# icameling/lidar_camera_calibration

Measured on AMD Instinct MI355X. Metric: chessboard-corner frames/sec + max corner error (mm), VLP-16 cloud, higher is better.
Workload: dtype f32

## Files before the change

lidar_camera_calibration_amd/csrc/ilcc_internal.h:

```cpp
#pragma once

#include <hip/hip_runtime.h>
#include <stdint.h>

#include "ilcc_hip.h"

#define ILCC_WAVE 64

namespace ilcc {

constexpr int kCropThreads = 256;
constexpr int kCropChunk = 4096;
#ifndef ILCC_K2_THREADS
#define ILCC_K2_THREADS 256
#endif
constexpr int kFrameThreads = ILCC_K2_THREADS;
#ifndef ILCC_K3_THREADS
#define ILCC_K3_THREADS 256
#endif
#ifndef ILCC_K45_THREADS
#define ILCC_K45_THREADS 256
#endif
constexpr int kPlaneThreads = ILCC_K3_THREADS;
constexpr int kPlaneThreadsSmallBatch = 1024;
#ifndef ILCC_SMALL_BATCH
#define ILCC_SMALL_BATCH 64
#endif
constexpr int kSmallBatchFrames = ILCC_SMALL_BATCH;
constexpr int kHistThreads = ILCC_K45_THREADS;
constexpr int kWalkThreads = 256;
#ifndef ILCC_K6_THREADS
#define ILCC_K6_THREADS 256
#endif
constexpr int kGridThreads = ILCC_K6_THREADS;
#ifndef ILCC_K6_THREADS_LARGE
#define ILCC_K6_THREADS_LARGE 512
#endif
constexpr int kGridThreadsLarge = ILCC_K6_THREADS_LARGE;
#ifndef ILCC_K6_LARGE_FROM
#define ILCC_K6_LARGE_FROM 2048
#endif
constexpr int kGridLargeFrom = ILCC_K6_LARGE_FROM;
constexpr int kTileA = 4;
#ifndef ILCC_TILE_B
#define ILCC_TILE_B 4
#endif
constexpr int kTileB = ILCC_TILE_B;
#ifndef ILCC_K6_GROUP
#define ILCC_K6_GROUP 7
#endif
constexpr int kThetaGroup = ILCC_K6_GROUP;
constexpr int kGridLdsPointsMax = 8192;
constexpr int kGridTableMax = 8192;
#ifndef ILCC_K7_THREADS
#define ILCC_K7_THREADS 256
#endif
constexpr int kSolveThreads = ILCC_K7_THREADS;
#ifndef ILCC_K7R_THREADS
#define ILCC_K7R_THREADS 192
#endif
constexpr int kRefineThreads = ILCC_K7R_THREADS;
constexpr int kRefineThreadsSmallBatch = 768;
constexpr int kRefineList = 32;
constexpr int kTieCap = 256;
constexpr float kTieEps = 2e-5f;
constexpr int kCoverageCellsMax = 1024;
constexpr int kIterSlots = 64;
constexpr int kBatchWords = 3 * kIterSlots + 2;
constexpr int kClusterHashSize = 1 << 17;
constexpr int kClusterLdsPointsMax = 4096;
constexpr int kClusterLdsPointsMin = 1024;
constexpr int kClusterCellsMin = 512;
constexpr int kClusterCellsMax = 6144;

struct GridPartial {
  float cost;
  uint32_t d2;
  uint32_t flat;
  uint32_t pad;
};

struct SolveRec {
  double x[3];
  double cost_a, cost_b, sel;
  double margin;
  int32_t iters_a, iters_b, phase, valid;
  int32_t flags, ties;
};

struct RefineOut {
  long long cost_q, alt_q;
  int32_t lat[3];
  int32_t phase, rounds, hops;
};

struct GridTables {
  const float* cth;
  const float* sth;
  const float* ay;
  const float* az;
  int32_t n_th, n_ty, n_tz;
  int32_t c_th, c_ty, c_tz;
};

struct SeedMap {
  int32_t stride_t, stride_th, off_th;
};

struct GridSeed {
  const GridPartial* records;
  uint32_t blocks;
  SeedMap map;
};

struct GridPass {
  GridTables t;
  GridPartial* out;
  uint32_t blocks;
  uint32_t walk_limit;
  uint32_t* bound;
  GridSeed seed;
  int32_t window_tiles, radius_th, step_th;
  uint32_t collect_ties;
  uint32_t box_points;
  uint32_t* grp_alive;
  uint32_t* grp_mask;
  uint32_t grp_count, grp_words;
};

struct Ctx {
  const float4* xyzi;
  const uint64_t* off;
  const float* clicks;
  uint32_t n_frames;
  uint32_t crop_chunks;
  ilcc_result* res;
  float4* roi;
  float4* cluster;
  float4* board;
  float4* pca;
  float4* optim;
  float2* yz;
  uint8_t* lab;
  uint32_t* n_lab;
  uint32_t* walk_stride;
  float2* walk_yz;
  uint8_t* walk_lab;
  uint32_t *walk_mi, *walk_nrim;
  uint8_t* cls;
  uint32_t* crop_counts;
  unsigned long long* crop_masks;
  uint32_t* uf_parent;
  uint32_t* uf_count;
  uint32_t* uf_hash_head;
  uint32_t* uf_hash_next;
  uint32_t cluster_lds_points;
  uint32_t cluster_cells_cap;
  uint32_t wide;
  uint32_t cluster_bits;
  uint32_t online_tier;
  float online_window;
  uint32_t* frame_flags;
  uint32_t* n_finite;
  uint32_t* crop_fin;
  uint32_t* list_count;
  uint32_t* list;
  void* list_frames;
  uint32_t list_grid;
  GridPartial* partial;
  SolveRec* solve_rec;
  uint32_t grid_blocks;
  uint32_t grid_lds_points;
  uint32_t* grid_bound;
  uint32_t* grid_bound_sub;
  uint32_t* tie_count;
  GridPartial* tie_list;
  unsigned long long* grid_iters;
  GridTables grid;
  const double2* th_lattice;
  int32_t th_lat_lo, th_lat_hi;
  int32_t refine_hop_y, refine_hop_z;
  ilcc_params p;
};

__host__ __device__ inline uint32_t walk_stride(uint32_t M) {
  if (M <= 2) return 1u;
  uint32_t S = ((uint32_t)((float)M * 0.6180339f)) | 1u;
  for (;; S += 2u) {
    uint32_t a = S, b = M;
    while (b) {
      const uint32_t t = a % b;
      a = b;
      b = t;
    }
    if (a == 1u) break;
  }
  return S >= M ? 1u : S;
}

__device__ __forceinline__ int lane_id() { return threadIdx.x & (ILCC_WAVE - 1); }
__device__ __forceinline__ int wave_id() { return threadIdx.x >> 6; }

template <typename T>
__device__ __forceinline__ T wave_sum(T v) {
#pragma unroll
  for (int o = ILCC_WAVE / 2; o > 0; o >>= 1) v += __shfl_down(v, o, ILCC_WAVE);
  return v;
}

template <typename T>
__device__ __forceinline__ T block_sum(T v, T* scratch) {
  v = wave_sum(v);
  const int nw = (blockDim.x + ILCC_WAVE - 1) / ILCC_WAVE;
  __syncthreads();
  if (lane_id() == 0) scratch[wave_id()] = v;
  __syncthreads();
// ... 90 lines not shown
```

lidar_camera_calibration_amd/csrc/k7_refine_corners.hip:

```cpp
#include "ilcc_internal.h"

namespace ilcc {

struct Divisor {
  double d, y;
};
__device__ __forceinline__ Divisor make_divisor(double d) { return Divisor{d, 1.0 / d}; }
__device__ __forceinline__ double div_by(double a, const Divisor& v) {
  const double q = a * v.y;
  const double r = __builtin_fma(-q, v.d, a);
  return __builtin_fma(r, v.y, q);
}

struct Board {
  double W, H, g, delta;
};
struct SolveBoard {
  double W, H, delta;
  double Wg2, Hg2;
  Divisor g;
};
__device__ __forceinline__ SolveBoard make_board(const ilcc_params& p) {
  SolveBoard b;
  b.W = (double)p.board_w;
// ... 531 lines not shown
      if (rel < 0.25) s.radius *= 0.5;
      if (rel > 0.75) s.radius = fmax(s.radius, 3.0 * s.step_norm);
      if (s.radius > 1e16) s.radius = 1e16;
      s.mu = fmax(1e-8, 2.0 * s.mu / 10.0);
      s.reuse = 0;
    } else {
      s.radius *= 0.5;
      s.reuse = 1;
    }
  }
  final_cost = x_cost;
  return iter;
}

__device__ __forceinline__ bool partial_less(const GridPartial& a, const GridPartial& b) {
  return a.cost < b.cost || (a.cost == b.cost && (a.d2 < b.d2 || (a.d2 == b.d2 && a.flat < b.flat)));
}

template <bool WIDE>
__device__ __forceinline__ void solve_wave(const Ctx& c, Problem& q, uint32_t f, uint32_t slot, SolveRec* out, Dog& dog) {
  double x[3] = {0.0, 0.0, 0.0};
  int phase = (int)slot;
  if (c.p.phase_mode != 2) {
    phase = (c.p.phase_mode == 1) ? 1 : 0;
  }
  q.tlw = phase != 0;
  double cost[2] = {0.0, 0.0};
  int iters[2] = {0, 0};
#pragma nounroll
  for (int pass = 0; pass < 2; ++pass) {
    q.oob = pass == 0;
    double fc = 0.0;
    const int it = trust_region_minimize<WIDE>(q, x, fc, c.p.max_iterations, dog);
    cost[pass] = fc;
    iters[pass] = it;
  }
#ifdef ILCC_K7_TIMING
  if (blockIdx.x == 0 && threadIdx.x == 0) {
    printf("K7a f0 slot %d: iters %d + %d; cycles dogleg %llu, evaluate<false> %llu, evaluate<true> %llu\n", (int)slot, iters[0], iters[1], g_k7_t[0], g_k7_t[1], g_k7_t[2]);
    g_k7_t[0] = g_k7_t[1] = g_k7_t[2] = 0;
  }
#endif
  q.oob = true;
  double cs[10];
  evaluate<false, WIDE>(q, x, cs);
  if (WIDE ? threadIdx.x == 0 : lane_id() == 0) {
    out->x[0] = x[0];
    out->x[1] = x[1];
    out->x[2] = x[2];
    out->cost_a = cost[0];
    out->cost_b = cost[1];
    out->sel = cs[0];
    out->iters_a = iters[0];
    out->iters_b = iters[1];
    out->phase = phase;
    out->valid = 1;
    out->margin = 0.0;
    out->flags = 0;
    out->ties = 0;
  }
}

#ifndef ILCC_K7A_WAVES_PER_EU
#define ILCC_K7A_WAVES_PER_EU 3
#endif
__global__ __launch_bounds__(kSolveThreads) __attribute__((amdgpu_waves_per_eu(ILCC_K7A_WAVES_PER_EU, ILCC_K7A_WAVES_PER_EU))) void k7a_local_solve(Ctx c, SolveRec* rec, int n_slots) {
  extern __shared__ __align__(16) unsigned char smem[];
  __shared__ Dog s_dog[kSolveWaves];
  const uint32_t wave = (uint32_t)wave_id();
  const uint32_t solve = blockIdx.x * (uint32_t)kSolveWaves + wave;
  const uint32_t f = solve / (uint32_t)n_slots, slot = solve % (uint32_t)n_slots;
  const bool live = f < c.n_frames && c.res[f].status == ILCC_OK;
  const uint32_t n = live ? c.n_lab[f] : 0u;
  const bool in_lds = n <= c.grid_lds_points;
  const uint32_t local_frame = wave / (uint32_t)n_slots;
  float2* s_yz = reinterpret_cast<float2*>(smem) + (size_t)local_frame * c.grid_lds_points;
  uint8_t* s_lab = smem + sizeof(float2) * (size_t)c.grid_lds_points * (size_t)(kSolveWaves / n_slots) + (size_t)local_frame * c.grid_lds_points;
  const uint64_t beg = live ? c.off[f] : 0u;
  if (live && in_lds) {
    for (uint32_t i = slot * ILCC_WAVE + (uint32_t)lane_id(); i < n; i += (uint32_t)n_slots * ILCC_WAVE) {
      s_yz[i] = c.yz[beg + i];
      s_lab[i] = c.lab[beg + i];
    }
  }
  __syncthreads();
  if (f >= c.n_frames) return;
  SolveRec* out = &rec[2 * f + slot];
  if (!live) {
    if (lane_id() == 0) out->valid = 0;
    return;
  }
  Problem q;
  q.n = n;
  q.bd = make_board(c.p);
  if (in_lds) {
    q.yz = s_yz;
    q.lab = s_lab;
    solve_wave<false>(c, q, f, slot, out, s_dog[wave]);
  } else {
    q.yz = c.yz + beg;
    q.lab = c.lab + beg;
    solve_wave<false>(c, q, f, slot, out, s_dog[wave]);
  }
}

__global__ __launch_bounds__(kSolveThreads) void k7a_local_solve_wide(Ctx c, SolveRec* rec) {
  extern __shared__ __align__(16) unsigned char smem[];
  __shared__ double s_red[2 * kSolveRedDoubles];
  __shared__ Dog s_dog[kSolveWaves];
  const uint32_t f = blockIdx.x, slot = blockIdx.y;
  SolveRec* out = &rec[2 * f + slot];
  if (c.res[f].status != ILCC_OK) {
    if (threadIdx.x == 0) out->valid = 0;
    return;
  }
  float2* s_yz = reinterpret_cast<float2*>(smem);
  uint8_t* s_lab = smem + sizeof(float2) * (size_t)c.grid_lds_points;
  const uint64_t beg = c.off[f];
  const uint32_t n = c.n_lab[f];
  int flip = 0;
  Problem q;
  q.n = n;
  q.bd = make_board(c.p);
  q.red = s_red;
  q.flip = &flip;
  if (n <= c.grid_lds_points) {
    for (uint32_t i = threadIdx.x; i < n; i += blockDim.x) {
      s_yz[i] = c.yz[beg + i];
      s_lab[i] = c.lab[beg + i];
    }
    __syncthreads();
    q.yz = s_yz;
    q.lab = s_lab;
    solve_wave<true>(c, q, f, slot, out, s_dog[wave_id()]);
  } else {
    q.yz = c.yz + beg;
    q.lab = c.lab + beg;
    solve_wave<true>(c, q, f, slot, out, s_dog[wave_id()]);
  }
}

constexpr double kCostQOne = 1099511627776.0;
#define kRefineWaves ((int)(blockDim.x >> 6))
static_assert(kRefineThreads % ILCC_WAVE == 0 && kRefineThreads / ILCC_WAVE >= 3 && kRefineThreads >= kRefineList &&
              kRefineThreadsSmallBatch % (3 * ILCC_WAVE) == 0,
              "ILCC_K7R_THREADS must be a multiple of 64, at least 192");
constexpr float kBorderRisk = 4e-6f;
constexpr int32_t kNoTheta = INT32_MIN;

struct RCand {
  int32_t q0, q1, q2, phase;
};
constexpr int kRefineWavesMax = kRefineThreadsSmallBatch / ILCC_WAVE;
constexpr int kActQueue = 128;
struct RefineShared {
  RCand cand[kRefineList];
  GridPartial meta[kRefineList];
  unsigned long long acc[3][kRefineList];
  uint32_t queue[kRefineWavesMax][kActQueue];
};

struct RefineState {
  int32_t lat[3];
  int32_t phase, rounds, hops, capped;
  int32_t skip_first;
  long long cost, alt;
};

struct AxisTerms {
  double in_dist;
  double out_dist;
  bool inside;
  bool odd;
};
__device__ __forceinline__ AxisTerms axis_terms(double v, double n) {
  AxisTerms t;
  t.inside = v > 0 && v < n;
  const double fl = floor(v);
  t.odd = (((int)fl) & 1) != 0;
  const double fr = v - fl;
  t.in_dist = (fr > 0.5) ? (fl + 1.0) - v : fr;
  t.out_dist = fmin(fabs(v), fabs(v - n));
  return t;
}
__device__ __forceinline__ double term_q(const AxisTerms& ai, const AxisTerms& aj, bool tlw, bool laser_white, double delta) {
#ifndef ILCC_K7R_BRANCHFREE
#define ILCC_K7R_BRANCHFREE 0
#endif
  double res = 0.0;
  if (ILCC_K7R_BRANCHFREE) {
    const bool white = tlw != (ai.odd != aj.odd);
    const double in_sum = ai.in_dist + aj.in_dist, out_sum = ai.out_dist + aj.out_dist;
    res = (ai.inside && aj.inside) ? ((laser_white != white) ? in_sum : 0.0) : out_sum;
  } else if (ai.inside && aj.inside) {
    const bool white = (ai.odd == aj.odd) ? tlw : !tlw;
    if (laser_white != white) res = ai.in_dist + aj.in_dist;
  } else {
    res = ai.out_dist + aj.out_dist;
  }
  const double r0 = (res > delta) ? 2.0 * delta * res - delta * delta : res * res;
  return rint(r0 * (0.5 * kCostQOne));
}

__device__ __forceinline__ int refine_sweep(const Ctx& c, const Board& bd, const float2* yz, const uint8_t* lab, uint32_t n,
                                            RefineShared& sh, int n_cand, int& sweep) {
  const int buf = sweep % 3;
  if (threadIdx.x < kRefineList) sh.acc[(sweep + 1) % 3][threadIdx.x] = 0ull;
  __syncthreads();
  const int lane = lane_id();
  const int slices = ILCC_WAVE / n_cand;
  const int cand = lane % n_cand, slice = lane / n_cand;
  if (slice < slices) {
    const RCand cd = sh.cand[cand];
    if (cd.q0 != kNoTheta) {
      const double div = (double)(c.p.refine_div > 0 ? c.p.refine_div : 1);
      const double2 cs = c.th_lattice[cd.q0 - c.th_lat_lo];
      const double x1 = c.p.ty_min + (double)cd.q1 * (c.p.ty_step / div), x2 = c.p.tz_min + (double)cd.q2 * (c.p.tz_step / div);
      const double inv_g = 1.0 / bd.g;
      const bool tlw = cd.phase != 0;
      long long sum = 0;
      for (uint32_t p = (uint32_t)(wave_id() * slices + slice); p < n; p += (uint32_t)(kRefineWaves * slices)) {
        const float2 v = yz[p];
        const double y = (double)v.x, z = (double)v.y;
        const double ry = cs.x * y - cs.y * z;
        const double rz = cs.y * y + cs.x * z;
        const AxisTerms ai = axis_terms(((ry + x1) + bd.W * bd.g / 2.0) * inv_g, bd.W);
        const AxisTerms aj = axis_terms(((rz + x2) + bd.H * bd.g / 2.0) * inv_g, bd.H);
        sum += (long long)term_q(ai, aj, tlw, lab[p] != 0, bd.delta);
      }
      atomicAdd(&sh.acc[buf][cand], (unsigned long long)sum);
    }
  }
  __syncthreads();
  ++sweep;
  return buf;
}

__device__ __forceinline__ int stencil_sweep(const Ctx& c, const Board& bd, const float2* yz, const uint8_t* lab, uint32_t n,
                                             RefineShared& sh, int n_th, const int32_t th[3], const int32_t ty[3],
                                             const int32_t tz[3], int phase, bool parity, int& sweep) {
  const int buf = sweep % 3;
  if (threadIdx.x < kRefineList) sh.acc[(sweep + 1) % 3][threadIdx.x] = 0ull;
  __syncthreads();
  const int wid = __builtin_amdgcn_readfirstlane(wave_id());
  const int waves_per_theta = kRefineWaves / n_th;
  const int it = wid % n_th, grp = wid / n_th;
  const int32_t q0 = th[it];
  if (grp < waves_per_theta && q0 != kNoTheta) {
    const int lane = lane_id();
    const double div = (double)(c.p.refine_div > 0 ? c.p.refine_div : 1);
    const double2 cs = c.th_lattice[q0 - c.th_lat_lo];
    double x1[3], x2[3];
#pragma unroll
    for (int k = 0; k < 3; ++k) {
      x1[k] = c.p.ty_min + (double)ty[k] * (c.p.ty_step / div);
      x2[k] = c.p.tz_min + (double)tz[k] * (c.p.tz_step / div);
    }
    const double inv_g = 1.0 / bd.g;
    double acc[9];
#pragma unroll
    for (int e = 0; e < 9; ++e) acc[e] = 0.0;
    auto eval_point = [&](uint32_t p) {
      const float2 v = yz[p];
      const bool laser_white = lab[p] != 0;
      const double y = (double)v.x, z = (double)v.y;
      const double ry = cs.x * y - cs.y * z;
      const double rz = cs.y * y + cs.x * z;
      AxisTerms ai[3], aj[3];
#pragma unroll
      for (int k = 0; k < 3; ++k) {
        ai[k] = axis_terms(((ry + x1[k]) + bd.W * bd.g / 2.0) * inv_g, bd.W);
        aj[k] = axis_terms(((rz + x2[k]) + bd.H * bd.g / 2.0) * inv_g, bd.H);
      }
#pragma unroll
      for (int a = 0; a < 3; ++a)
#pragma unroll
        for (int b = 0; b < 3; ++b) {
          const bool tlw = ((phase ^ (parity ? ((a + b) & 1) : 0)) != 0);
          acc[a * 3 + b] += term_q(ai[a], aj[b], tlw, laser_white, bd.delta);
        }
    };
    const uint32_t n_slices = (uint32_t)(waves_per_theta * ILCC_WAVE);
    const bool skip_silent = !parity && ty[0] <= ty[1] && ty[1] <= ty[2] && tz[0] <= tz[1] && tz[1] <= tz[2] && c.p.ty_step > 0.0 && c.p.tz_step > 0.0;
    if (skip_silent) {
      uint32_t* queue = sh.queue[wid];
      uint32_t head = 0, tail = 0;
      const bool tlw0 = phase != 0;
      for (uint32_t base = (uint32_t)(grp * ILCC_WAVE); base < n; base += n_slices) {
        const uint32_t p = base + (uint32_t)lane;
        bool active = false;
        if (p < n) {
          const float2 v = yz[p];
          const double y = (double)v.x, z = (double)v.y;
          const double ry = cs.x * y - cs.y * z;
          const double rz = cs.y * y + cs.x * z;
          const double i0 = ((ry + x1[0]) + bd.W * bd.g / 2.0) * inv_g, i2 = ((ry + x1[2]) + bd.W * bd.g / 2.0) * inv_g;
          const double j0 = ((rz + x2[0]) + bd.H * bd.g / 2.0) * inv_g, j2 = ((rz + x2[2]) + bd.H * bd.g / 2.0) * inv_g;
          const double fi = floor(i0), fj = floor(j0);
          const bool one_cell = i0 > 0 && i2 < bd.W && j0 > 0 && j2 < bd.H && fi == floor(i2) && fj == floor(j2);
          const bool odd_i = (((int)fi) & 1) != 0, odd_j = (((int)fj) & 1) != 0;
          const bool white = (odd_i == odd_j) ? tlw0 : !tlw0;
          active = !(one_cell && (lab[p] != 0) == white);
        }
        const unsigned long long m = __ballot(active);
        if (m != 0ull) {
          if (active) queue[(tail + (uint32_t)__popcll(m & ((1ull << lane) - 1ull))) & (kActQueue - 1)] = p;
          tail += (uint32_t)__popcll(m);
          __builtin_amdgcn_fence(__ATOMIC_RELEASE, "wavefront");
          __builtin_amdgcn_wave_barrier();
          __builtin_amdgcn_fence(__ATOMIC_ACQUIRE, "wavefront");
          while (tail - head >= (uint32_t)ILCC_WAVE) {
            eval_point(queue[(head + (uint32_t)lane) & (kActQueue - 1)]);
            head += ILCC_WAVE;
          }
          __builtin_amdgcn_fence(__ATOMIC_RELEASE, "wavefront");
          __builtin_amdgcn_wave_barrier();
        }
      }
      if ((uint32_t)lane < tail - head) eval_point(queue[(head + (uint32_t)lane) & (kActQueue - 1)]);
    } else {
      for (uint32_t p = (uint32_t)(grp * ILCC_WAVE + lane); p < n; p += n_slices) eval_point(p);
    }
#pragma unroll
    for (int e = 0; e < 9; ++e) {
      unsigned long long t = (unsigned long long)(long long)acc[e];
      t += xor_lane_u64<8>(t);
      t += xor_lane_u64<4>(t);
      t += xor_lane_u64<2>(t);
      t += xor_lane_u64<1>(t);
      if ((lane & 15) == 0) atomicAdd(&sh.acc[buf][it * 9 + e], t);
    }
  }
  __syncthreads();
  ++sweep;
  return buf;
}

__device__ void pattern_refine(const Ctx& c, const Board& bd, const float2* yz, const uint8_t* lab, uint32_t n,
                               RefineShared& sh, int& sweep, RefineState& st) {
  const bool refine = c.p.refine_div > 0;
  const int div = refine ? c.p.refine_div : 1;
  st.rounds = 0;
  st.hops = 0;
  st.capped = 0;
  st.cost = 0;
  st.alt = 0;
  for (;;) {
    int stride = div, r = 0;
    if (st.skip_first && refine && div >= 2 && c.p.refine_max_rounds >= 1) {
      stride = div >> 1;
      r = 1;
    }
    st.skip_first = 0;
    while (refine && stride >= 1 && r < c.p.refine_max_rounds) {
      int32_t th[3], ty[3], tz[3];
#pragma unroll
      for (int k = 0; k < 3; ++k) {
        const int q0 = st.lat[0] + (k - 1) * stride;
        th[k] = (q0 < c.th_lat_lo || q0 > c.th_lat_hi) ? kNoTheta : q0;
        ty[k] = st.lat[1] + (k - 1) * stride;
        tz[k] = st.lat[2] + (k - 1) * stride;
      }
      const int b = stencil_sweep(c, bd, yz, lab, n, sh, 3, th, ty, tz, st.phase, false, sweep);
      long long bc = LLONG_MAX;
      int bd2 = 0, be = -1;
      for (int e = 0; e < 27; ++e) {
        if (e == 13) continue;
        const int dk = e / 9 - 1, da = (e / 3) % 3 - 1, db = e % 3 - 1;
        const int q0 = st.lat[0] + dk * stride;
        if (q0 < c.th_lat_lo || q0 > c.th_lat_hi) continue;
        const long long cc = (long long)sh.acc[b][e];
        const int d2 = dk * dk + da * da + db * db;
        if (cc < bc || (cc == bc && d2 < bd2)) {
          bc = cc;
          bd2 = d2;
          be = e;
        }
      }
      const long long centre = (long long)sh.acc[b][13];
      ++r;
      if (be >= 0 && bc < centre) {
        st.lat[0] += (be / 9 - 1) * stride;
        st.lat[1] += ((be / 3) % 3 - 1) * stride;
        st.lat[2] += (be % 3 - 1) * stride;
      } else {
        stride >>= 1;
      }
    }
    st.rounds += r;
    if (refine && stride >= 1) st.capped = 1;
    const int32_t th1[3] = {st.lat[0], kNoTheta, kNoTheta};
    const int32_t hy[3] = {st.lat[1] - c.refine_hop_y, st.lat[1], st.lat[1] + c.refine_hop_y};
    const int32_t hz[3] = {st.lat[2] - c.refine_hop_z, st.lat[2], st.lat[2] + c.refine_hop_z};
    const int b = stencil_sweep(c, bd, yz, lab, n, sh, 1, th1, hy, hz, st.phase, true, sweep);
    st.cost = (long long)sh.acc[b][4];
    long long alt = LLONG_MAX;
    int ae = -1;
    for (int e = 0; e < 9; ++e) {
      if (e == 4) continue;
      const long long cc = (long long)sh.acc[b][e];
      if (cc < alt) {
        alt = cc;
        ae = e;
      }
    }
    st.alt = alt;
    if (alt < st.cost && st.hops < 2 && refine) {
      const int da = ae / 3 - 1, db = ae % 3 - 1;
      ++st.hops;
      st.lat[1] += da * c.refine_hop_y;
      st.lat[2] += db * c.refine_hop_z;
      st.phase ^= (da + db) & 1;
      continue;
    }
    break;
  }
}

template <bool LDS_POINTS>
__device__ void refine_frame(const Ctx& c, SolveRec* rec, float2* s_yz, uint8_t* s_lab, RefineShared& sh) {
  const uint32_t f = blockIdx.x;
  ilcc_result* r = &c.res[f];
  SolveRec* out = &rec[2 * f];
  const int lane = lane_id(), tid = (int)threadIdx.x;
  const uint64_t beg = c.off[f];
  const uint32_t n = c.n_lab[f];
  const Board bd{(double)c.p.board_w, (double)c.p.board_h, c.p.grid_length, c.p.huber_delta};
  const float2* yz = c.yz + beg;
  const uint8_t* lab = c.lab + beg;
  if (tid < kRefineList) sh.acc[0][tid] = 0ull;
  if (LDS_POINTS) {
    for (uint32_t i = threadIdx.x; i < n; i += blockDim.x) {
      s_yz[i] = yz[i];
      s_lab[i] = lab[i];
    }
    yz = s_yz;
    lab = s_lab;
  }
  __syncthreads();

  const GridPartial* gp = c.partial + (uint64_t)f * c.grid_blocks;
  GridPartial b{__builtin_inff(), 0xFFFFFFFFu, 0xFFFFFFFFu, 0u};
  for (uint32_t k = lane; k < c.grid_blocks; k += ILCC_WAVE) {
    const GridPartial t = gp[k];
    if (partial_less(t, b)) b = t;
  }
#pragma unroll
  for (int o = ILCC_WAVE / 2; o > 0; o >>= 1) {
    GridPartial t;
    t.cost = __shfl_xor(b.cost, o, ILCC_WAVE);
    t.d2 = __shfl_xor(b.d2, o, ILCC_WAVE);
    t.flat = __shfl_xor(b.flat, o, ILCC_WAVE);
    if (partial_less(t, b)) b = t;
  }
  if (b.flat == 0xFFFFFFFFu) {
    if (tid == 0) out->valid = 0;
    return;
  }
  int sweep = 0;
  int flags = 0;
  uint32_t n_ties = 0;
  const int div = c.p.refine_div > 0 ? c.p.refine_div : 1;
  const uint32_t n_ty = (uint32_t)c.p.n_ty, n_tz = (uint32_t)c.p.n_tz;
  if (c.tie_count != nullptr) {
    n_ties = c.tie_count[f];
    if (n_ties > (uint32_t)kTieCap) {
      flags |= ILCC_FLAG_TIE_OVERFLOW;
    } else {
      const GridPartial* tl = c.tie_list + (uint64_t)f * kTieCap;
      const float window = b.cost * (1.f + kTieEps);
      uint32_t close = 0;
      for (uint32_t e = 0; e < n_ties; ++e) close += (tl[e].cost <= window && tl[e].flat != b.flat) ? 1u : 0u;
      if (close > 0) {
        long long best_q = LLONG_MAX;
        GridPartial pick = b;
        int k = 0;
        for (uint32_t e = 0; e <= n_ties; ++e) {
          const GridPartial t = (e < n_ties) ? tl[e] : b;
          const bool take = (t.cost <= window) && !(e < n_ties && t.flat == b.flat);
          if (take) {
            if (tid == 0) {
              const uint32_t cl = t.flat >> 1;
              sh.cand[k] = RCand{(int32_t)(cl / (n_tz * n_ty)) * div, (int32_t)((cl / n_tz) % n_ty) * div, (int32_t)(cl % n_tz) * div, (int32_t)(t.flat & 1u)};
              sh.meta[k] = t;
            }
            ++k;
          }
          if (k == kRefineList || (e == n_ties && k > 0)) {
            const int bf = refine_sweep(c, bd, yz, lab, n, sh, k, sweep);
            for (int j = 0; j < k; ++j) {
              const long long cq = (long long)sh.acc[bf][j];
              const GridPartial m = sh.meta[j];
              if (cq < best_q || (cq == best_q && (m.d2 < pick.d2 || (m.d2 == pick.d2 && m.flat < pick.flat)))) {
                best_q = cq;
                pick = m;
              }
            }
            k = 0;
            __syncthreads();
          }
        }
        b = pick;
      }
    }
  }
  if (tid == 0) {
    r->grid_index = (int32_t)b.flat;
    r->grid_cost = b.cost;
  }
  const uint32_t cell = b.flat >> 1;
  RefineState st;
  st.lat[0] = (int32_t)(cell / (n_tz * n_ty)) * div;
  st.lat[1] = (int32_t)((cell / n_tz) % n_ty) * div;
  st.lat[2] = (int32_t)(cell % n_tz) * div;
  st.phase = (int)(b.flat & 1u);
#ifndef ILCC_K7R_SKIP_FIRST
#define ILCC_K7R_SKIP_FIRST 1
#endif
  {
    const int gk = (int)(cell / (n_tz * n_ty)), ga = (int)((cell / n_tz) % n_ty), gb = (int)(cell % n_tz);
    bool risk = false;
    for (uint32_t i = (uint32_t)tid; i < n; i += blockDim.x) {
      const float2 v = yz[i];
#pragma unroll
      for (int dk = -1; dk <= 1; ++dk) {
        const int k = gk + dk;
        if (k < 0 || k >= c.p.n_th) continue;
        const float cth = c.grid.cth[k], sth = c.grid.sth[k];
        const float pi = fmaf(-sth, v.y, cth * v.x), pj = fmaf(cth, v.y, sth * v.x);
#pragma unroll
        for (int d = -1; d <= 1; ++d) {
          const int a = ga + d, b = gb + d;
          if (a >= 0 && a < (int)n_ty) {
            const float x = pi + c.grid.ay[a];
            risk |= fabsf(x - rintf(x)) < kBorderRisk;
          }
          if (b >= 0 && b < (int)n_tz) {
            const float x = pj + c.grid.az[b];
            risk |= fabsf(x - rintf(x)) < kBorderRisk;
          }
        }
      }
    }
    risk = __syncthreads_or(risk ? 1 : 0) != 0;
    if (risk) flags |= ILCC_FLAG_BORDER_RISK;
    st.skip_first = ILCC_K7R_SKIP_FIRST && !risk && !(flags & ILCC_FLAG_TIE_OVERFLOW) && gk > 0 && gk < c.p.n_th - 1 && ga > 0 &&
                    ga < (int)n_ty - 1 && gb > 0 && gb < (int)n_tz - 1;
  }
  pattern_refine(c, bd, yz, lab, n, sh, sweep, st);
  if (tid == 0) {
    const double dv = (double)div;
    out->x[0] = c.p.th_min + (double)st.lat[0] * (c.p.th_step / dv);
    out->x[1] = c.p.ty_min + (double)st.lat[1] * (c.p.ty_step / dv);
    out->x[2] = c.p.tz_min + (double)st.lat[2] * (c.p.tz_step / dv);
    out->cost_a = out->sel = (double)st.cost / kCostQOne;
    out->cost_b = (double)st.alt / kCostQOne;
    out->margin = ((double)st.alt - (double)st.cost) / (double)(st.cost > 0 ? st.cost : 1);
    out->iters_a = st.rounds;
    out->iters_b = st.hops;
    out->phase = st.phase;
    out->valid = 1;
    out->flags = flags | (st.capped ? ILCC_FLAG_REFINE_CAPPED : 0);
    out->ties = (int32_t)n_ties;
  }
}

__global__ __launch_bounds__(kRefineThreadsSmallBatch) void k7r_pattern_refine(Ctx c, SolveRec* rec) {
  extern __shared__ __align__(16) unsigned char smem[];
  __shared__ RefineShared sh;
  const uint32_t f = blockIdx.x;
  if (c.res[f].status != ILCC_OK) {
    if (threadIdx.x == 0) rec[2 * f].valid = 0;
    return;
  }
  float2* s_yz = reinterpret_cast<float2*>(smem);
  uint8_t* s_lab = smem + sizeof(float2) * (size_t)c.grid_lds_points;
  if (c.n_lab[f] <= c.grid_lds_points)
    refine_frame<true>(c, rec, s_yz, s_lab, sh);
  else
    refine_frame<false>(c, rec, s_yz, s_lab, sh);
}

__global__ __launch_bounds__(kRefineThreads) void k7r_pattern_refine_test(Ctx c, RefineOut* io) {
  __shared__ RefineShared sh;
  if (threadIdx.x < kRefineList) sh.acc[0][threadIdx.x] = 0ull;
  __syncthreads();
  const Board bd{(double)c.p.board_w, (double)c.p.board_h, c.p.grid_length, c.p.huber_delta};
  RefineState st;
  st.lat[0] = io->lat[0];
  st.lat[1] = io->lat[1];
  st.lat[2] = io->lat[2];
  st.phase = io->phase;
  st.skip_first = 0;
  int sweep = 0;
  __syncthreads();
  pattern_refine(c, bd, c.yz, c.lab, c.n_lab[0], sh, sweep, st);
  if (threadIdx.x == 0) {
    io->lat[0] = st.lat[0];
    io->lat[1] = st.lat[1];
    io->lat[2] = st.lat[2];
    io->phase = st.phase;
    io->rounds = st.rounds;
    io->hops = st.hops;
    io->cost_q = st.cost;
    io->alt_q = st.alt;
  }
}

__device__ __forceinline__ void inv_rigid_apply(const float* T, const float in[3], float out[3]) {
  const float dx = in[0] - T[3], dy = in[1] - T[7], dz = in[2] - T[11];
#pragma unroll
  for (int c = 0; c < 3; ++c) {
    float s = T[0 + c] * dx;
    s = s + T[4 + c] * dy;
    s = s + T[8 + c] * dz;
    out[c] = s;
  }
}

__global__ __launch_bounds__(kSolveThreads) void k7b_corners(Ctx c, const SolveRec* rec, int n_slots) {
  __shared__ float s_T[16];
  __shared__ uint32_t s_hit[kCoverageCellsMax / 32];
  __shared__ uint32_t s_oob;
  const uint32_t f = blockIdx.x;
  ilcc_result* r = &c.res[f];
  if (r->status != ILCC_OK) return;
  const uint32_t tid = threadIdx.x;
  const uint64_t beg = c.off[f];
  SolveRec best = rec[2 * f];
  if (n_slots > 1) {
    const SolveRec o = rec[2 * f + 1];
    if (o.valid && (!best.valid || o.sel < best.sel)) best = o;
  }
  if (!best.valid) {
    if (tid == 0) r->status = ILCC_BAD_ARGUMENT;
    return;
  }
  if (tid == 0) {
    r->theta_t[0] = best.x[0];
    r->theta_t[1] = best.x[1];
    r->theta_t[2] = best.x[2];
    r->cost_a = best.cost_a;
    r->cost_b = best.cost_b;
    r->sel_cost = best.sel;
    r->phase = best.phase;
    r->iters_a = best.iters_a;
    r->iters_b = best.iters_b;
    r->basin_margin = best.margin;
    r->flags = best.flags;
    r->grid_ties = best.ties;
    const float roll = (float)best.x[0];
    const float E = cosf(roll), F = sinf(roll);
    const float T[16] = {1, 0, 0, 0, 0, E, -F, (float)best.x[1], 0, F, E, (float)best.x[2], 0, 0, 0, 1};
    for (int k = 0; k < 16; ++k) s_T[k] = T[k];
    s_oob = 0u;
  }
  for (int k = (int)tid; k < kCoverageCellsMax / 32; k += kSolveThreads) s_hit[k] = 0u;
  __syncthreads();

  const int W = c.p.board_w, H = c.p.board_h;
  {
    const double g = c.p.grid_length, ct = cos(best.x[0]), st = sin(best.x[0]);
    const uint32_t nl = c.n_lab[f];
    const float2* __restrict__ yz = c.yz + beg;
    uint32_t oob = 0;
    for (uint32_t k = tid; k < nl; k += kSolveThreads) {
      const float2 v = yz[k];
      const double yy = ct * (double)v.x - st * (double)v.y + best.x[1];
      const double zz = st * (double)v.x + ct * (double)v.y + best.x[2];
      const double i = (yy + W * g / 2.0) / g, j = (zz + H * g / 2.0) / g;
      if (i > 0.0 && i < (double)W && j > 0.0 && j < (double)H) {
        const int cell = (int)floor(i) * H + (int)floor(j);
        atomicOr(&s_hit[cell >> 5], 1u << (cell & 31));
      } else {
        ++oob;
      }
    }
    if (oob) atomicAdd(&s_oob, oob);
    __syncthreads();
    if (tid == 0) {
      int cells = 0;
      for (int k = 0; k < (W * H + 31) / 32; ++k) cells += __popc(s_hit[k]);
      r->cells_hit = cells;
      r->n_oob = (int32_t)s_oob;
      if (c.p.min_cell_coverage > 0.0 && (double)cells < c.p.min_cell_coverage * (double)(W * H)) r->flags = best.flags | ILCC_FLAG_LOW_COVERAGE;
    }
  }
  const int nc = (W - 1) * (H - 1);
  const int ncc = nc < ILCC_MAX_CORNERS ? nc : ILCC_MAX_CORNERS;
  for (int t = (int)tid; t < ncc; t += kSolveThreads) {
    const int i = 1 + t / (H - 1), j = 1 + t % (H - 1);
    const double xg = (i - (double)W / 2.0) * c.p.grid_length;
    const double yg = (j - (double)H / 2.0) * c.p.grid_length;
    const float pt[3] = {0.0f, (float)xg, (float)yg};
    float a[3], w[3];
    inv_rigid_apply(s_T, pt, a);
    inv_rigid_apply(r->pca, a, w);
    r->corners[3 * t] = w[0];
    r->corners[3 * t + 1] = w[1];
    r->corners[3 * t + 2] = w[2];
  }
  if (tid == 0) r->n_corners = ncc;

  const uint32_t M = (uint32_t)r->n_plane;
  const float4* __restrict__ Q = c.pca + beg;
  float4* __restrict__ O = c.optim + beg;
  for (uint32_t i = tid; i < M; i += kSolveThreads) {
    const float4 v = Q[i];
    float o[3];
#pragma unroll
    for (int rr = 0; rr < 3; ++rr) {
      float s = s_T[4 * rr] * v.x;
      s = s + s_T[4 * rr + 1] * v.y;
      s = s + s_T[4 * rr + 2] * v.z;
      s = s + s_T[4 * rr + 3];
      o[rr] = s;
    }
    O[i] = make_float4(o[0], o[1], o[2], v.w);
  }
  __syncthreads();
  if (tid == 0 && c.p.solver == ILCC_SOLVER_GRID && c.p.ambiguity_eps > 0.0 && best.margin < c.p.ambiguity_eps) r->status = ILCC_AMBIGUOUS;
}

__global__ __launch_bounds__(ILCC_WAVE) void k7_local_solve_test(Ctx c, int tlw, int use_oob, double* theta_t,
                                                                 double* cost_iters) {
  Problem q;
  q.yz = c.yz;
  q.lab = c.lab;
  q.n = c.n_lab[0];
  q.bd = make_board(c.p);
  q.tlw = tlw != 0;
  q.oob = use_oob != 0;
  __shared__ Dog s_dog1;
  double x[3] = {theta_t[0], theta_t[1], theta_t[2]};
  double cost = 0;
  const int it = trust_region_minimize<false>(q, x, cost, c.p.max_iterations, s_dog1);
  if (threadIdx.x == 0) {
    theta_t[0] = x[0];
    theta_t[1] = x[1];
    theta_t[2] = x[2];
    cost_iters[0] = cost;
    cost_iters[1] = (double)it;
  }
}

hipError_t set_kernel_attributes_k7() {
  const int cap = (int)((sizeof(float2) + 1) * (size_t)kGridLdsPointsMax);
  hipError_t e = hipFuncSetAttribute((const void*)k7a_local_solve, hipFuncAttributeMaxDynamicSharedMemorySize, kSolveLdsMax);
  if (e == hipSuccess) e = hipFuncSetAttribute((const void*)k7a_local_solve_wide, hipFuncAttributeMaxDynamicSharedMemorySize, cap);
  if (e == hipSuccess) e = hipFuncSetAttribute((const void*)k7r_pattern_refine, hipFuncAttributeMaxDynamicSharedMemorySize, cap);
  return e;
}

void launch_pattern_refine_corners(const Ctx& c, hipStream_t s) {
  const size_t lds = (sizeof(float2) + 1) * (size_t)c.grid_lds_points;
  const int threads = c.n_frames <= (uint32_t)kSmallBatchFrames ? kRefineThreadsSmallBatch : kRefineThreads;
  hipLaunchKernelGGL(k7r_pattern_refine, dim3(c.n_frames), dim3(threads), lds, s, c, c.solve_rec);
  hipLaunchKernelGGL(k7b_corners, dim3(c.n_frames), dim3(kSolveThreads), 0, s, c, c.solve_rec, 1);
}

void launch_pattern_refine_test(const Ctx& c, hipStream_t s, RefineOut* d_io) {
  hipLaunchKernelGGL(k7r_pattern_refine_test, dim3(1), dim3(kRefineThreads), 0, s, c, d_io);
}

void launch_refine_corners(const Ctx& c, hipStream_t s) {
  const int n_slots = (c.p.solver == ILCC_SOLVER_REFERENCE_LOCAL && c.p.phase_mode == 2) ? 2 : 1;
  if (c.n_frames <= (uint32_t)kSolveWideMaxFrames) {
    const size_t lds1 = (sizeof(float2) + 1) * (size_t)c.grid_lds_points;
    hipLaunchKernelGGL(k7a_local_solve_wide, dim3(c.n_frames, n_slots), dim3(kSolveThreads), lds1, s, c, c.solve_rec);
    hipLaunchKernelGGL(k7b_corners, dim3(c.n_frames), dim3(kSolveThreads), 0, s, c, c.solve_rec, n_slots);
    return;
  }
  Ctx ck = c;
  size_t lds = (sizeof(float2) + 1) * (size_t)c.grid_lds_points * (size_t)(kSolveWaves / n_slots);
  if (lds > (size_t)kSolveLdsMax) {
    ck.grid_lds_points = 0;
    lds = 0;
  }
  const uint32_t solves = c.n_frames * (uint32_t)n_slots;
  hipLaunchKernelGGL(k7a_local_solve, dim3((solves + kSolveWaves - 1) / kSolveWaves), dim3(kSolveThreads), lds, s, ck, c.solve_rec, n_slots);
  hipLaunchKernelGGL(k7b_corners, dim3(c.n_frames), dim3(kSolveThreads), 0, s, c, c.solve_rec, n_slots);
}

void launch_local_solve(const Ctx& c, hipStream_t s, int32_t tlw, int32_t use_oob, double* theta_t,
                        double* cost_iters) {
  hipLaunchKernelGGL(k7_local_solve_test, dim3(1), dim3(ILCC_WAVE), 0, s, c, tlw, use_oob, theta_t, cost_iters);
}

__global__ __launch_bounds__(128) void k9_pack_records(const ilcc_result* __restrict__ res, uint32_t n_corners, uint32_t tag_base,
                                                       float* __restrict__ out) {
  __shared__ uint32_t s_x[2];
  const ilcc_result& r = res[blockIdx.x];
  const uint32_t width = (uint32_t)ILCC_RECORD_HEADER + 3u * n_corners;
  float* o = out + (uint64_t)blockIdx.x * width;
  const uint32_t have = (uint32_t)(r.n_corners < 0 ? 0 : r.n_corners);
  const uint32_t tag = (tag_base + blockIdx.x) & 0xFFFFFFu;
  uint32_t x = 0;
  for (uint32_t k = threadIdx.x; k < width; k += blockDim.x) {
    float v = 0.f;
    if (k >= (uint32_t)ILCC_RECORD_HEADER) {
      const uint32_t c = k - (uint32_t)ILCC_RECORD_HEADER;
      v = (c < 3u * have) ? r.corners[c] : 0.f;
      x ^= __float_as_uint(v) * (2u * c + 1u);
    } else {
      switch (k) {
        case 0: v = (float)r.status; break;
        case 1: v = (float)r.n_corners; break;
        case 2: v = (float)r.phase; break;
        case 3: v = (float)r.grid_index; break;
        case 4: v = (float)r.iters_a; break;
        case 5: v = (float)r.iters_b; break;
        case 6: v = (float)r.cost_a; break;
        case 7: v = (float)r.cost_b; break;
        case 8: v = (float)r.sel_cost; break;
        case 9: v = (float)r.theta_t[0]; break;
        case 10: v = (float)r.theta_t[1]; break;
        case 11: v = (float)r.theta_t[2]; break;
        case 12: v = (float)r.n_plane; break;
        case 13: v = (float)r.n_black; break;
        case 14: v = (float)r.n_white; break;
        case 15: v = (float)r.basin_margin; break;
        case 16: v = (float)tag; break;
        case 18: v = (float)r.flags; break;
        case 19: v = (float)r.n_roi; break;
        default: v = 0.f;
      }
    }
    if (k != 17u) o[k] = v;
  }
#pragma unroll
  for (int of = ILCC_WAVE / 2; of > 0; of >>= 1) x ^= __shfl_xor(x, of, ILCC_WAVE);
  if ((threadIdx.x & (ILCC_WAVE - 1)) == 0) s_x[threadIdx.x >> 6] = x;
  __syncthreads();
  if (threadIdx.x == 0) {
    uint32_t t = s_x[0] ^ s_x[1] ^ (tag * 0x9E3779B1u);
    t = (t ^ (t >> 24)) & 0xFFFFFFu;
    o[17] = (float)t;
  }
}

__global__ __launch_bounds__(256) void k_store_to_host(const uint32_t* __restrict__ src, uint32_t* __restrict__ host_dst, uint32_t n_words) {
  for (uint32_t i = blockIdx.x * blockDim.x + threadIdx.x; i < n_words; i += gridDim.x * blockDim.x) host_dst[i] = src[i];
}
void launch_store_to_host(const void* d_src, void* h_dst, size_t bytes, hipStream_t s) {
  const uint32_t n_words = (uint32_t)(bytes / 4);
  if (n_words == 0) return;
  const uint32_t blocks = std::min<uint32_t>(256u, (n_words + 255u) / 256u);
  hipLaunchKernelGGL(k_store_to_host, dim3(blocks), dim3(256), 0, s, static_cast<const uint32_t*>(d_src), static_cast<uint32_t*>(h_dst), n_words);
}

void launch_pack_records(const ilcc_result* d_res, uint32_t n_frames, uint32_t n_corners, uint32_t tag_base, float* d_out,
                         hipStream_t s) {
  if (n_frames) hipLaunchKernelGGL(k9_pack_records, dim3(n_frames), dim3(128), 0, s, d_res, n_corners, tag_base, d_out);
}

}
```

Before: 1.302 million.

## Prefilter refine points into per-wave LDS candidate lists over a lattice window

Adds a window filter that, for a lattice window around the current refine position, drops points that provably stay in one same-coloured cell over the whole window. It stores the survivors as uint16 indices in per-wave LDS segments, and later stencil sweeps iterate only those lists instead of all points. The window is narrowed and re-filtered as the search converges. The serial 27- and 9-candidate argmin scans are replaced by lane-parallel shuffle reductions. The cost is extra dynamic LDS per block, which may lower occupancy, plus refilter passes and fallback logic when a segment overflows.

```diff
diff --git a/lidar_camera_calibration_amd/csrc/ilcc_internal.h b/lidar_camera_calibration_amd/csrc/ilcc_internal.h
--- a/lidar_camera_calibration_amd/csrc/ilcc_internal.h
+++ b/lidar_camera_calibration_amd/csrc/ilcc_internal.h
@@ -62,6 +62,10 @@
 constexpr int kRefineThreads = ILCC_K7R_THREADS;
 constexpr int kRefineThreadsSmallBatch = 768;
 constexpr int kRefineList = 32;
+constexpr int kActQueue = 128;
+constexpr int kRefineTestList = 2112;
+constexpr int kRefineListPointsMax = 65535;
+constexpr uint32_t refine_list_segment(uint32_t points, uint32_t waves) { return 64u * (((points + 63u) / 64u + waves - 1u) / waves); }
 constexpr int kTieCap = 256;
 constexpr float kTieEps = 2e-5f;
 constexpr int kCoverageCellsMax = 1024;
diff --git a/lidar_camera_calibration_amd/csrc/k7_refine_corners.hip b/lidar_camera_calibration_amd/csrc/k7_refine_corners.hip
--- a/lidar_camera_calibration_amd/csrc/k7_refine_corners.hip
+++ b/lidar_camera_calibration_amd/csrc/k7_refine_corners.hip
@@ -707,12 +707,33 @@
   int32_t q0, q1, q2, phase;
 };
 constexpr int kRefineWavesMax = kRefineThreadsSmallBatch / ILCC_WAVE;
-constexpr int kActQueue = 128;
 struct RefineShared {
   RCand cand[kRefineList];
   GridPartial meta[kRefineList];
   unsigned long long acc[3][kRefineList];
-  uint32_t queue[kRefineWavesMax][kActQueue];
+  uint32_t list_n[kRefineWavesMax];
+};
+struct RefineLds {
+  uint32_t* queue;
+  uint16_t* list;
+  uint32_t seg_cap;
+};
+__host__ __device__ constexpr size_t refine_lds_bytes(uint32_t waves, uint32_t list_points) {
+  return sizeof(uint32_t) * kActQueue * waves + sizeof(uint16_t) * (size_t)refine_list_segment(list_points, waves) * waves;
+}
+__device__ __forceinline__ RefineLds make_refine_lds(unsigned char* at, uint32_t list_points, uint32_t n) {
+  const uint32_t waves = (uint32_t)(blockDim.x >> 6);
+  RefineLds l;
+  l.queue = reinterpret_cast<uint32_t*>(at);
+  l.seg_cap = refine_list_segment(list_points, waves);
+  l.list = (list_points != 0u && n <= (uint32_t)kRefineListPointsMax) ? reinterpret_cast<uint16_t*>(at + sizeof(uint32_t) * kActQueue * waves) : nullptr;
+  return l;
+}
+
+struct RefineWindow {
+  int32_t c[3], hw, phase;
+  bool have;
+  bool full;
 };
 
 struct RefineState {
@@ -791,12 +812,65 @@
   return buf;
 }
 
+
+__device__ __forceinline__ void window_filter(const Ctx& c, const Board& bd, const float2* yz, const uint8_t* lab, uint32_t n,
+                                              RefineShared& sh, const RefineLds& lds, const RefineWindow& w, bool narrow) {
+  const int wid = __builtin_amdgcn_readfirstlane(wave_id());
+  const int lane = lane_id();
+  const double div = (double)(c.p.refine_div > 0 ? c.p.refine_div : 1);
+  const double2 cs = c.th_lattice[w.c[0] - c.th_lat_lo];
+  const double x1lo = c.p.ty_min + (double)(w.c[1] - w.hw) * (c.p.ty_step / div), x1hi = c.p.ty_min + (double)(w.c[1] + w.hw) * (c.p.ty_step / div);
+  const double x2lo = c.p.tz_min + (double)(w.c[2] - w.hw) * (c.p.tz_step / div), x2hi = c.p.tz_min + (double)(w.c[2] + w.hw) * (c.p.tz_step / div);
+  const double inv_g = 1.0 / bd.g;
+  const double dth = (double)w.hw * fabs(c.p.th_step) / div;
+  const bool tlw0 = w.phase != 0;
+  uint16_t* seg = lds.list + (size_t)wid * lds.seg_cap;
+  const uint32_t lim = narrow ? min(sh.list_n[wid], lds.seg_cap) : n;
+  const uint32_t step = narrow ? (uint32_t)ILCC_WAVE : (uint32_t)(kRefineWaves * ILCC_WAVE);
+  uint32_t count = 0;
+  for (uint32_t base = narrow ? 0u : (uint32_t)(wid * ILCC_WAVE); base < lim; base += step) {
+    const uint32_t k = base + (uint32_t)lane;
+    uint32_t p = k;
+    if (narrow && k < lim) p = seg[k];
+    bool keep = false;
+    if (k < lim) {
+      const float2 v = yz[p];
+      const double y = (double)v.x, z = (double)v.y;
+      const double ry = cs.x * y - cs.y * z;
+      const double rz = cs.y * y + cs.x * z;
+      const double rho = sqrt(y * y + z * z) * (1.0 + 1e-12);
+      const double m = rho * dth * inv_g * (1.0 + 1e-9) + 1e-9;
+      const double i0 = ((ry + x1lo) + bd.W * bd.g / 2.0) * inv_g - m, i2 = ((ry + x1hi) + bd.W * bd.g / 2.0) * inv_g + m;
+      const double j0 = ((rz + x2lo) + bd.H * bd.g / 2.0) * inv_g - m, j2 = ((rz + x2hi) + bd.H * bd.g / 2.0) * inv_g + m;
+      const double fi = floor(i0), fj = floor(j0);
+      const bool one_cell = i0 > 0 && i2 < bd.W && j0 > 0 && j2 < bd.H && fi == floor(i2) && fj == floor(j2);
+      const bool odd_i = (((int)fi) & 1) != 0, odd_j = (((int)fj) & 1) != 0;
+      const bool white = (odd_i == odd_j) ? tlw0 : !tlw0;
+      keep = !(one_cell && (lab[p] != 0) == white);
+    }
+    const unsigned long long mk = __ballot(keep);
+    const uint32_t at = count + (uint32_t)__popcll(mk & ((1ull << lane) - 1ull));
+    if (keep && at < lds.seg_cap) seg[at] = (uint16_t)p;
+    count += (uint32_t)__popcll(mk);
+  }
+  if (lane == 0) sh.list_n[wid] = count;
+}
+
 __device__ __forceinline__ int stencil_sweep(const Ctx& c, const Board& bd, const float2* yz, const uint8_t* lab, uint32_t n,
-                                             RefineShared& sh, int n_th, const int32_t th[3], const int32_t ty[3],
-                                             const int32_t tz[3], int phase, bool parity, int& sweep) {
+                                             RefineShared& sh, const RefineLds& lds, bool windowed, bool& win_full, int n_th, const int32_t th[3],
+                                             const int32_t ty[3], const int32_t tz[3], int phase, bool parity, int& sweep) {
   const int buf = sweep % 3;
   if (threadIdx.x < kRefineList) sh.acc[(sweep + 1) % 3][threadIdx.x] = 0ull;
   __syncthreads();
+  bool use_list = false;
+  if (windowed) {
+    if (!win_full) {
+      bool over = false;
+      for (int k = 0; k < kRefineWaves; ++k) over |= sh.list_n[k] > lds.seg_cap;
+      win_full = over;
+    }
+    use_list = !win_full;
+  }
   const int wid = __builtin_amdgcn_readfirstlane(wave_id());
   const int waves_per_theta = kRefineWaves / n_th;
   const int it = wid % n_th, grp = wid / n_th;
@@ -838,38 +912,45 @@
     const uint32_t n_slices = (uint32_t)(waves_per_theta * ILCC_WAVE);
     const bool skip_silent = !parity && ty[0] <= ty[1] && ty[1] <= ty[2] && tz[0] <= tz[1] && tz[1] <= tz[2] && c.p.ty_step > 0.0 && c.p.tz_step > 0.0;
     if (skip_silent) {
-      uint32_t* queue = sh.queue[wid];
+      uint32_t* queue = lds.queue + wid * kActQueue;
       uint32_t head = 0, tail = 0;
       const bool tlw0 = phase != 0;
-      for (uint32_t base = (uint32_t)(grp * ILCC_WAVE); base < n; base += n_slices) {
-        const uint32_t p = base + (uint32_t)lane;
-        bool active = false;
-        if (p < n) {
-          const float2 v = yz[p];
-          const double y = (double)v.x, z = (double)v.y;
-          const double ry = cs.x * y - cs.y * z;
-          const double rz = cs.y * y + cs.x * z;
-          const double i0 = ((ry + x1[0]) + bd.W * bd.g / 2.0) * inv_g, i2 = ((ry + x1[2]) + bd.W * bd.g / 2.0) * inv_g;
-          const double j0 = ((rz + x2[0]) + bd.H * bd.g / 2.0) * inv_g, j2 = ((rz + x2[2]) + bd.H * bd.g / 2.0) * inv_g;
-          const double fi = floor(i0), fj = floor(j0);
-          const bool one_cell = i0 > 0 && i2 < bd.W && j0 > 0 && j2 < bd.H && fi == floor(i2) && fj == floor(j2);
-          const bool odd_i = (((int)fi) & 1) != 0, odd_j = (((int)fj) & 1) != 0;
-          const bool white = (odd_i == odd_j) ? tlw0 : !tlw0;
-          active = !(one_cell && (lab[p] != 0) == white);
-        }
-        const unsigned long long m = __ballot(active);
-        if (m != 0ull) {
-          if (active) queue[(tail + (uint32_t)__popcll(m & ((1ull << lane) - 1ull))) & (kActQueue - 1)] = p;
-          tail += (uint32_t)__popcll(m);
-          __builtin_amdgcn_fence(__ATOMIC_RELEASE, "wavefront");
-          __builtin_amdgcn_wave_barrier();
-          __builtin_amdgcn_fence(__ATOMIC_ACQUIRE, "wavefront");
-          while (tail - head >= (uint32_t)ILCC_WAVE) {
-            eval_point(queue[(head + (uint32_t)lane) & (kActQueue - 1)]);
-            head += ILCC_WAVE;
+      const int n_seg = use_list ? kRefineWaves : 1;
+      for (int sg = use_list ? grp : 0; sg < n_seg; sg += waves_per_theta) {
+        const uint16_t* seg = use_list ? lds.list + (size_t)sg * lds.seg_cap : nullptr;
+        const uint32_t lim = use_list ? sh.list_n[sg] : n, step = use_list ? (uint32_t)ILCC_WAVE : n_slices;
+        for (uint32_t base = use_list ? 0u : (uint32_t)(grp * ILCC_WAVE); base < lim; base += step) {
+          const uint32_t k = base + (uint32_t)lane;
+          uint32_t p = k;
+          if (use_list && k < lim) p = seg[k];
+          bool active = false;
+          if (k < lim) {
+            const float2 v = yz[p];
+            const double y = (double)v.x, z = (double)v.y;
+            const double ry = cs.x * y - cs.y * z;
+            const double rz = cs.y * y + cs.x * z;
+            const double i0 = ((ry + x1[0]) + bd.W * bd.g / 2.0) * inv_g, i2 = ((ry + x1[2]) + bd.W * bd.g / 2.0) * inv_g;
+            const double j0 = ((rz + x2[0]) + bd.H * bd.g / 2.0) * inv_g, j2 = ((rz + x2[2]) + bd.H * bd.g / 2.0) * inv_g;
+            const double fi = floor(i0), fj = floor(j0);
+            const bool one_cell = i0 > 0 && i2 < bd.W && j0 > 0 && j2 < bd.H && fi == floor(i2) && fj == floor(j2);
+            const bool odd_i = (((int)fi) & 1) != 0, odd_j = (((int)fj) & 1) != 0;
+            const bool white = (odd_i == odd_j) ? tlw0 : !tlw0;
+            active = !(one_cell && (lab[p] != 0) == white);
           }
-          __builtin_amdgcn_fence(__ATOMIC_RELEASE, "wavefront");
-          __builtin_amdgcn_wave_barrier();
+          const unsigned long long m = __ballot(active);
+          if (m != 0ull) {
+            if (active) queue[(tail + (uint32_t)__popcll(m & ((1ull << lane) - 1ull))) & (kActQueue - 1)] = p;
+            tail += (uint32_t)__popcll(m);
+            __builtin_amdgcn_fence(__ATOMIC_RELEASE, "wavefront");
+            __builtin_amdgcn_wave_barrier();
+            __builtin_amdgcn_fence(__ATOMIC_ACQUIRE, "wavefront");
+            while (tail - head >= (uint32_t)ILCC_WAVE) {
+              eval_point(queue[(head + (uint32_t)lane) & (kActQueue - 1)]);
+              head += ILCC_WAVE;
+            }
+            __builtin_amdgcn_fence(__ATOMIC_RELEASE, "wavefront");
+            __builtin_amdgcn_wave_barrier();
+          }
         }
       }
       if ((uint32_t)lane < tail - head) eval_point(queue[(head + (uint32_t)lane) & (kActQueue - 1)]);
@@ -891,10 +972,33 @@
   return buf;
 }
 
+__device__ __forceinline__ void lanes_argmin(long long& cost, uint32_t& tag) {
+  auto step = [&](unsigned long long oc, uint32_t ot) {
+    const bool take = (long long)oc < cost || ((long long)oc == cost && ot < tag);
+    cost = take ? (long long)oc : cost;
+    tag = take ? ot : tag;
+  };
+  step(xor_lane_u64<16>((unsigned long long)cost), xor_lane_u32<16>(tag));
+  step(xor_lane_u64<8>((unsigned long long)cost), xor_lane_u32<8>(tag));
+  step(xor_lane_u64<4>((unsigned long long)cost), xor_lane_u32<4>(tag));
+  step(xor_lane_u64<2>((unsigned long long)cost), xor_lane_u32<2>(tag));
+  step(xor_lane_u64<1>((unsigned long long)cost), xor_lane_u32<1>(tag));
+  const uint32_t lo = (uint32_t)__builtin_amdgcn_readfirstlane((int)(uint32_t)(unsigned long long)cost);
+  const uint32_t hi = (uint32_t)__builtin_amdgcn_readfirstlane((int)(uint32_t)((unsigned long long)cost >> 32));
+  cost = (long long)(((unsigned long long)hi << 32) | lo);
+  tag = (uint32_t)__builtin_amdgcn_readfirstlane((int)tag);
+}
+
 __device__ void pattern_refine(const Ctx& c, const Board& bd, const float2* yz, const uint8_t* lab, uint32_t n,
-                               RefineShared& sh, int& sweep, RefineState& st) {
+                               RefineShared& sh, const RefineLds& lds, int& sweep, RefineState& st) {
   const bool refine = c.p.refine_div > 0;
   const int div = refine ? c.p.refine_div : 1;
+  const int lane = lane_id();
+  const bool listed = lds.list != nullptr && c.p.ty_step > 0.0 && c.p.tz_step > 0.0;
+  RefineWindow win;
+  win.c[0] = win.c[1] = win.c[2] = win.hw = win.phase = 0;
+  win.have = false;
+  win.full = false;
   st.rounds = 0;
   st.hops = 0;
   st.capped = 0;
@@ -916,22 +1020,39 @@
         ty[k] = st.lat[1] + (k - 1) * stride;
         tz[k] = st.lat[2] + (k - 1) * stride;
       }
-      const int b = stencil_sweep(c, bd, yz, lab, n, sh, 3, th, ty, tz, st.phase, false, sweep);
-      long long bc = LLONG_MAX;
-      int bd2 = 0, be = -1;
-      for (int e = 0; e < 27; ++e) {
-        if (e == 13) continue;
-        const int dk = e / 9 - 1, da = (e / 3) % 3 - 1, db = e % 3 - 1;
-        const int q0 = st.lat[0] + dk * stride;
-        if (q0 < c.th_lat_lo || q0 > c.th_lat_hi) continue;
-        const long long cc = (long long)sh.acc[b][e];
-        const int d2 = dk * dk + da * da + db * db;
-        if (cc < bc || (cc == bc && d2 < bd2)) {
-          bc = cc;
-          bd2 = d2;
-          be = e;
+      if (listed) {
+        bool inside = win.have && win.phase == st.phase, nested = inside;
+#pragma unroll
+        for (int k = 0; k < 3; ++k) {
+          const int off = abs(st.lat[k] - win.c[k]);
+          inside = inside && off + stride <= win.hw;
+          nested = nested && off + 2 * stride <= win.hw;
+        }
+        const bool narrow = inside && nested && !win.full && win.hw >= 4 * stride;
+        if (!inside || narrow) {
+          win.c[0] = st.lat[0];
+          win.c[1] = st.lat[1];
+          win.c[2] = st.lat[2];
+          win.hw = 2 * stride;
+          win.phase = st.phase;
+          win.have = true;
+          win.full = false;
+          window_filter(c, bd, yz, lab, n, sh, lds, win, narrow);
         }
       }
+      const int b = stencil_sweep(c, bd, yz, lab, n, sh, lds, listed, win.full, 3, th, ty, tz, st.phase, false, sweep);
+      long long bc = LLONG_MAX;
+      uint32_t btag = 0xFFFFFFFFu;
+      if (lane < 27 && lane != 13) {
+        const int dk = lane / 9 - 1, da = (lane / 3) % 3 - 1, db = lane % 3 - 1;
+        const int q0 = st.lat[0] + dk * stride;
+        if (q0 >= c.th_lat_lo && q0 <= c.th_lat_hi) {
+          bc = (long long)sh.acc[b][lane];
+          btag = ((uint32_t)(dk * dk + da * da + db * db) << 8) | (uint32_t)lane;
+        }
+      }
+      lanes_argmin(bc, btag);
+      const int be = (btag == 0xFFFFFFFFu) ? -1 : (int)(btag & 0xFFu);
       const long long centre = (long long)sh.acc[b][13];
       ++r;
       if (be >= 0 && bc < centre) {
@@ -947,25 +1068,24 @@
     const int32_t th1[3] = {st.lat[0], kNoTheta, kNoTheta};
     const int32_t hy[3] = {st.lat[1] - c.refine_hop_y, st.lat[1], st.lat[1] + c.refine_hop_y};
     const int32_t hz[3] = {st.lat[2] - c.refine_hop_z, st.lat[2], st.lat[2] + c.refine_hop_z};
-    const int b = stencil_sweep(c, bd, yz, lab, n, sh, 1, th1, hy, hz, st.phase, true, sweep);
+    const int b = stencil_sweep(c, bd, yz, lab, n, sh, lds, false, win.full, 1, th1, hy, hz, st.phase, true, sweep);
     st.cost = (long long)sh.acc[b][4];
     long long alt = LLONG_MAX;
-    int ae = -1;
-    for (int e = 0; e < 9; ++e) {
-      if (e == 4) continue;
-      const long long cc = (long long)sh.acc[b][e];
-      if (cc < alt) {
-        alt = cc;
-        ae = e;
-      }
-    }
+    uint32_t atag = 0xFFFFFFFFu;
+    if (lane < 9 && lane != 4) {
+      alt = (long long)sh.acc[b][lane];
+      atag = (uint32_t)lane;
+    }
+    lanes_argmin(alt, atag);
     st.alt = alt;
     if (alt < st.cost && st.hops < 2 && refine) {
+      const int ae = (int)atag;
       const int da = ae / 3 - 1, db = ae % 3 - 1;
       ++st.hops;
       st.lat[1] += da * c.refine_hop_y;
       st.lat[2] += db * c.refine_hop_z;
       st.phase ^= (da + db) & 1;
+      win.have = false;
       continue;
     }
     break;
@@ -973,7 +1093,7 @@
 }
 
 template <bool LDS_POINTS>
-__device__ void refine_frame(const Ctx& c, SolveRec* rec, float2* s_yz, uint8_t* s_lab, RefineShared& sh) {
+__device__ void refine_frame(const Ctx& c, SolveRec* rec, float2* s_yz, uint8_t* s_lab, RefineShared& sh, const RefineLds& lds) {
   const uint32_t f = blockIdx.x;
   ilcc_result* r = &c.res[f];
   SolveRec* out = &rec[2 * f];
@@ -1102,7 +1222,7 @@
     st.skip_first = ILCC_K7R_SKIP_FIRST && !risk && !(flags & ILCC_FLAG_TIE_OVERFLOW) && gk > 0 && gk < c.p.n_th - 1 && ga > 0 &&
                     ga < (int)n_ty - 1 && gb > 0 && gb < (int)n_tz - 1;
   }
-  pattern_refine(c, bd, yz, lab, n, sh, sweep, st);
+  pattern_refine(c, bd, yz, lab, n, sh, lds, sweep, st);
   if (tid == 0) {
     const double dv = (double)div;
     out->x[0] = c.p.th_min + (double)st.lat[0] * (c.p.th_step / dv);
@@ -1130,14 +1250,17 @@
   }
   float2* s_yz = reinterpret_cast<float2*>(smem);
   uint8_t* s_lab = smem + sizeof(float2) * (size_t)c.grid_lds_points;
-  if (c.n_lab[f] <= c.grid_lds_points)
-    refine_frame<true>(c, rec, s_yz, s_lab, sh);
+  unsigned char* behind = smem + (sizeof(float2) + 1) * (size_t)c.grid_lds_points;
+  const uint32_t n = c.n_lab[f];
+  if (n <= c.grid_lds_points)
+    refine_frame<true>(c, rec, s_yz, s_lab, sh, make_refine_lds(behind, c.grid_lds_points, n));
   else
-    refine_frame<false>(c, rec, s_yz, s_lab, sh);
+    refine_frame<false>(c, rec, s_yz, s_lab, sh, make_refine_lds(behind, 0u, n));
 }
 
 __global__ __launch_bounds__(kRefineThreads) void k7r_pattern_refine_test(Ctx c, RefineOut* io) {
   __shared__ RefineShared sh;
+  __shared__ __align__(4) unsigned char s_lds[refine_lds_bytes(kRefineThreads / ILCC_WAVE, kRefineTestList)];
   if (threadIdx.x < kRefineList) sh.acc[0][threadIdx.x] = 0ull;
   __syncthreads();
   const Board bd{(double)c.p.board_w, (double)c.p.board_h, c.p.grid_length, c.p.huber_delta};
@@ -1149,7 +1272,7 @@
   st.skip_first = 0;
   int sweep = 0;
   __syncthreads();
-  pattern_refine(c, bd, c.yz, c.lab, c.n_lab[0], sh, sweep, st);
+  pattern_refine(c, bd, c.yz, c.lab, c.n_lab[0], sh, make_refine_lds(s_lds, kRefineTestList, c.n_lab[0]), sweep, st);
   if (threadIdx.x == 0) {
     io->lat[0] = st.lat[0];
     io->lat[1] = st.lat[1];
@@ -1301,15 +1424,16 @@
 
 hipError_t set_kernel_attributes_k7() {
   const int cap = (int)((sizeof(float2) + 1) * (size_t)kGridLdsPointsMax);
+  const int cap_r = cap + (int)refine_lds_bytes(kRefineWavesMax, kGridLdsPointsMax);
   hipError_t e = hipFuncSetAttribute((const void*)k7a_local_solve, hipFuncAttributeMaxDynamicSharedMemorySize, kSolveLdsMax);
   if (e == hipSuccess) e = hipFuncSetAttribute((const void*)k7a_local_solve_wide, hipFuncAttributeMaxDynamicSharedMemorySize, cap);
-  if (e == hipSuccess) e = hipFuncSetAttribute((const void*)k7r_pattern_refine, hipFuncAttributeMaxDynamicSharedMemorySize, cap);
+  if (e == hipSuccess) e = hipFuncSetAttribute((const void*)k7r_pattern_refine, hipFuncAttributeMaxDynamicSharedMemorySize, cap_r);
   return e;
 }
 
 void launch_pattern_refine_corners(const Ctx& c, hipStream_t s) {
-  const size_t lds = (sizeof(float2) + 1) * (size_t)c.grid_lds_points;
   const int threads = c.n_frames <= (uint32_t)kSmallBatchFrames ? kRefineThreadsSmallBatch : kRefineThreads;
+  const size_t lds = (sizeof(float2) + 1) * (size_t)c.grid_lds_points + refine_lds_bytes((uint32_t)threads / ILCC_WAVE, c.grid_lds_points);
   hipLaunchKernelGGL(k7r_pattern_refine, dim3(c.n_frames), dim3(threads), lds, s, c, c.solve_rec);
   hipLaunchKernelGGL(k7b_corners, dim3(c.n_frames), dim3(kSolveThreads), 0, s, c, c.solve_rec, 1);
 }
```

Measured after the change: 1.344 million (median of 6 runs). 1.03x the previous value.
